# ffreyer/MonteCarlo.jl

Hardware: AMD Instinct MI355X
Metric: DQMC sweeps/sec, 16x16 Hubbard beta=8 dtau=0.1; achieved % fp64 MFMA roofline (higher is better)
Workload: dtype f64

## Files before the change

montecarlo.jl_amd/csrc/engine.cpp:

```cpp
#include <hip/hip_runtime.h>

#include <algorithm>
#include <cmath>
#include <cstdio>
#include <cstdlib>
#include <cstring>
#include <string>
#include <vector>

#include "../../include/dqmc_hip.h"
#include "kernels.h"
#include <rccl/rccl.h>

using namespace dqmc;

struct dqmc_comm {
    ncclComm_t comm = nullptr;
    int nranks = 1, rank = 0, device = 0;
};

static thread_local std::string g_create_error;

struct UTStack;

struct dqmc_handle {
    dqmc_params p{};
    int n = 0, nb = 1, N = 0, M = 0, s = 0, K = 0, W = 0, units = 0;
    long nn = 0;
    double lambda = 0, epl = 0, eml = 0;
    SweepConsts sc{};
    hipStream_t stream = nullptr;
    KernelSwitches sw;
    double *eT = nullptr, *eTinv = nullptr, *eT2 = nullptr, *eTinv2 = nullptr;
    double *eT2T = nullptr;
    bool slab = false;
    bool kron = false;
    double *kron_f = nullptr;
    int kron_fa = 0, kron_fb = 0;
    int8_t *conf = nullptr;
    double *u_stack = nullptr, *t_stack = nullptr, *d_stack = nullptr;
    std::vector<double *> su, sd, st;
    double *Ul = nullptr, *Ur = nullptr, *Tl = nullptr, *Tr = nullptr, *greens = nullptr, *greens_temp = nullptr;
    double *tmp1 = nullptr, *tmp2 = nullptr, *bufA = nullptr, *bufB = nullptr;
    struct QrSet {
        double *V = nullptr, *W = nullptr, *S = nullptr, *tau = nullptr, *winv = nullptr, *ts = nullptr;
        int *pivot = nullptr;
    } qs[1];
    double *&qrV = qs[0].V, *&qrW = qs[0].W, *&qrS = qs[0].S, *&trsm_w = qs[0].winv, *&trsm_s = qs[0].ts, *&tau = qs[0].tau;
    int *&pivot = qs[0].pivot;
    double *Dl = nullptr, *Dr = nullptr;
    hipStream_t cur = nullptr;
    double *greens_alt = nullptr, *lu_img = nullptr;
    bool sweep_fused = true;
    WalkerRng *rng = nullptr;
    DevStats *stats = nullptr;
    unsigned long long *pc_scratch = nullptr;
    std::vector<double *> uniforms;
    double *acc = nullptr;
    size_t acc_n = 0;
    int n_dirs = 0;
    int *dir_ptr = nullptr, *pair_src = nullptr, *pair_trg = nullptr;
    double *corr_per_walker = nullptr, *corr_acc = nullptr;
    int K_loc = 0;
    int *trg_of = nullptr;
    size_t pc_n = 0;
    double *pc_per_walker = nullptr, *pc_acc = nullptr;
    int K_cc = 0;
    std::vector<int> cc_trg_h;
    std::vector<double> cc_T;
    CCPlan cc;
    size_t corr_n = 0;
    int current_slice = 0, direction = 0;
    bool prepared = false;
    long long conf_version = 0;
    UTStack *ut = nullptr;
    std::string err;
    bool timing = false;
    struct Ev { hipEvent_t a, b; int fam; };
    std::vector<Ev> pending;
    std::vector<hipEvent_t> pool;
    double fam_ms[DQMC_K_COUNT] = {0};
    long long fam_n[DQMC_K_COUNT] = {0};
    std::vector<void *> allocs;
    QrCoopWorkspace qr_ws;
    int qrb_sites = 0;
    struct {
// ... 240 lines not shown
    auto exy = [&](int r, int c) {
        if (tr) std::swap(r, c);
        return fy[(r >> 3) + 8 * (c >> 3)] * fx[(r & 7) + 8 * (c & 7)];
    };
    auto ez = [&](int r, int c) { return tr ? fz[c + 8 * r] : fz[r + 8 * c]; };
    for (int mp = 0; mp < 4; ++mp)
        for (int m = 0; m < 4; ++m)
            for (int r = 0; r < 4; ++r)
                for (int lane = 0; lane < 64; ++lane)
                    img_xy[((mp * 4 + m) * 4 + r) * 64 + lane] = exy(16 * mp + (lane & 15), 16 * m + 4 * r + (lane >> 4));
    for (int q = 0; q < 4; ++q)
        for (int lane = 0; lane < 64; ++lane) {
            const int row = lane & 15, k = 4 * q + (lane >> 4);
            img_z[q * 64 + lane] = (row >> 3) == (k >> 3) ? ez(row & 7, k & 7) : 0.0;
        }
}

static void read_kernel_switches(dqmc_handle *h)
{
    KernelSwitches &k = h->sw;
    k.qr_noblocked = getenv("DQMC_QR_NOBLOCKED") != nullptr;
    if (const char *e = getenv("DQMC_QRB_SITES")) k.qrb_sites = atoi(e) & 7;
    if (const char *e = getenv("DQMC_QR_TAIL")) k.qr_tail = atoi(e) != 0;
    k.qr_sc1 = getenv("DQMC_QR_SC1") != nullptr;
    k.qr_nocoop = getenv("DQMC_QR_NOCOOP") != nullptr;
    if (const char *e = getenv("DQMC_QR_FORCE_TIMEOUT"))
        k.qr_force_timeout = strncmp(e, "step:", 5) == 0 ? 2 + atoi(e + 5) : (strncmp(e, "extra:", 6) == 0 ? 1000 + atoi(e + 6) : 1);
    k.qr_nopanel = getenv("DQMC_QR_NOPANEL") != nullptr;
    k.trsm_simple = getenv("DQMC_TRSM_SIMPLE") != nullptr;
    k.sweep_split = getenv("DQMC_SWEEP_SPLIT") != nullptr;
    k.flush_ncp2 = getenv("DQMC_FLUSH_NCP2") != nullptr;
    k.no_slab = getenv("DQMC_NO_SLAB") != nullptr;
    k.no_kron = getenv("DQMC_NO_KRON") != nullptr;
}

static int alloc_qr_workspace(dqmc_handle *h)
{
    CHK(dalloc(h, &h->qr_ws.errflag, (size_t)1));
    h->qr_ws.tail = h->sw.qr_tail;
    h->qr_ws.force_sc1 = h->sw.qr_sc1;
    h->qr_ws.no_coop = h->sw.qr_nocoop;
    h->qr_ws.no_panel = h->sw.qr_nopanel;
    h->qr_ws.force_timeout = h->sw.qr_force_timeout;
    if (h->n > 256) return 0;
    hipDeviceProp_t prop;
    HIPCHK(hipGetDeviceProperties(&prop, h->p.device_id));
    const size_t slots = (size_t)((h->units + 7) / 8) * 8 * QR_COOP_SLOTS_PER_UNIT;
    CHK(dalloc(h, &h->qr_ws.mailbox, slots * QR_COOP_SLOT));
    CHK(dalloc(h, &h->qr_ws.fb, (size_t)2));
    h->qr_ws.max_blocks = prop.multiProcessorCount * qr_coop_blocks_per_cu();
    h->qr_ws.epoch = 0;
    h->qrb_sites = 0;
    if (h->n == 256 && !h->sw.qr_noblocked) {
        const int per_cu = qrb_blocks_per_cu();
        if (per_cu >= 1 && ((h->units + 7) / 8) * 64 <= prop.multiProcessorCount * per_cu) {
            CHK(dalloc(h, (char **)&h->qr_ws.mailbox2, qrb_mailbox_bytes(h->units)));
            h->qr_ws.blk_max_blocks = prop.multiProcessorCount * per_cu;
            h->qrb_sites = h->sw.qrb_sites;
        }
    }
    return 0;
}
static int check_qr_workspace(dqmc_handle *h)
{
    if (!h->qr_ws.errflag) return 0;
    int e = 0;
// ... 144 lines not shown
static SlabArgs slab_base(dqmc_handle *h, const double *X0, long x_su, long x_sb, double *out)
{
    SlabArgs a{};
    a.n_units = h->units; a.nb = h->nb; a.nsteps = 0;
    a.X0 = X0; a.x_su = x_su; a.x_sb = x_sb;
    a.out = out; a.out_su = h->nn;
    a.conf_stride = (long)h->N * h->M;
    a.epl = h->epl; a.eml = h->eml;
    return a;
}
static void slab_step_const(dqmc_handle *h, SlabArgs &a, const double *C)
{
    SlabStep &st = a.st[a.nsteps++];
    st = SlabStep{};
    st.A = C; st.su = 0; st.sb = h->nn;
}
static void slab_step_unit(dqmc_handle *h, SlabArgs &a, const double *A)
{
    SlabStep &st = a.st[a.nsteps++];
    st = SlabStep{};
    st.A = A; st.su = h->nn; st.sb = 0;
}
static int run_slab(dqmc_handle *h, const SlabArgs &a)
{
    hipEvent_t ea, eb;
    timing_events(h, &ea, &eb);
    HIPCHK(launch_slab_chain(a, h->cur, ea, eb));
    return timing_push(h, ea, eb, DQMC_K_GEMM);
}

enum { KF_ET2 = 0, KF_ETINV2 = 1, KF_ET2T = 2, KF_ETINV2T = 3 };
static bool use_kron(const dqmc_handle *h) { return h->kron && !h->cb.on; }
static bool oop_wrap(const dqmc_handle *h) { return (h->slab || h->kron) && !h->cb.on; }
static KronArgs kron_base(dqmc_handle *h, const double *X0, double *out)
{
    KronArgs a{};
    a.n_units = h->units; a.nb = h->nb; a.nsteps = 0;
    a.X0 = X0; a.x_su = h->nn;
    a.out = out; a.out_su = h->nn;
    a.conf_stride = (long)h->N * h->M;
    a.epl = h->epl; a.eml = h->eml;
    return a;
}
static KronStep &kron_step(dqmc_handle *h, KronArgs &a, int which)
{
    KronStep &st = a.st[a.nsteps++];
    st = KronStep{};
    st.ax = h->kron_f + (size_t)which * h->nb * (h->kron_fa + h->kron_fb);
    st.ay = st.ax + (size_t)h->nb * h->kron_fa;
    return st;
}
static int run_kron(dqmc_handle *h, const KronArgs &a)
{
    hipEvent_t ea, eb;
    timing_events(h, &ea, &eb);
    if (h->n == 512) HIPCHK(launch_kron3_chain(a, h->cur, ea, eb));
    else HIPCHK(launch_kron_chain(a, h->cur, ea, eb));
    return timing_push(h, ea, eb, DQMC_K_GEMM);
}

static const int8_t *conf_slice(dqmc_handle *h, int slice) { return h->conf + (long)(slice - 1) * h->N; }
static void chain_steps(dqmc_handle *h, SlabArgs &a, int dir, int idx, int t0, int t1)
{
    for (int t = t0; t < t1; ++t) {
        SlabStep &st = a.st[a.nsteps];
        if (dir == 1) {
// ... 45 lines not shown
        const int slice = dir == 1 ? (idx - 1) * h->s + 1 + t : idx * h->s - t;
        out = (t & 1) ? h->bufB : h->bufA;
        if (h->cb.on) {
            CHK(cb_mult(h, dir == 1 ? CB_LEFT_B : CB_LEFT_BDAG, slice, X, out, t == h->s - 1 ? dslot(h, src) : nullptr));
            X = out;
            continue;
        }
        GemmArgs g = gemm_base(h, C_(h, h->eT2), dir == 1 ? 0 : 1, U_(h, X), 0, out);
        if (dir == 1) g.kscale = vs_conf(h, slice, +1);
        else { g.rowscale = vs_conf(h, slice, +1); g.row_first = 1; }
        if (t == h->s - 1) g.colscale = vs_arr(dslot(h, src), h->n);
        CHK(run_gemm(h, g));
        X = out;
    }
    const int sp = h->K + 1;
    if (udt_is_fused(h, 0)) {
        CHK(udt_fused(h, out, uslot(h, sp), dslot(h, sp), h->tmp2, 1, h->qs[0]));
    } else {
        CHK(udt_factor(h, out, dslot(h, sp), h->tmp2, 1, h->qs[0]));
        CHK(udt_formq(h, uslot(h, sp), h->qs[0], h->qs[0].winv, h->qs[0].ts));
    }
    CHK(run_gemm(h, gemm_base(h, U_(h, h->tmp2), 0, U_(h, tslot(h, src)), 0, tslot(h, sp))));
    slot_swap_spare(h, dst);
    return 0;
}
static int add_slice_sequence_left(dqmc_handle *h, int idx, bool wrap_temp = false) { return add_slice_sequence(h, +1, idx, wrap_temp); }
static int add_slice_sequence_right(dqmc_handle *h, int idx) { return add_slice_sequence(h, -1, idx, false); }

static int wrap_greens_kron(dqmc_handle *h, const double *src, double *dst, int curr_slice, int direction)
{
    const int8_t *c = conf_slice(h, direction == -1 ? curr_slice - 1 : curr_slice);
    KronArgs a = kron_base(h, src, h->bufB);
    a.transpose_out = 1;
    KronStep &s1 = kron_step(h, a, direction == -1 ? KF_ETINV2 : KF_ET2);
    if (direction == -1) { s1.post_conf = c; s1.post_sign = -1; }
    else { s1.pre_conf = c; s1.pre_sign = +1; }
    CHK(run_kron(h, a));
    KronArgs b = kron_base(h, h->bufB, dst);
    b.transpose_out = 1;
    KronStep &s2 = kron_step(h, b, direction == -1 ? KF_ET2T : KF_ETINV2T);
    if (direction == -1) { s2.post_conf = c; s2.post_sign = +1; }
    else { s2.pre_conf = c; s2.pre_sign = -1; }
    return run_kron(h, b);
}
static int wrap_greens_slab(dqmc_handle *h, const double *src, double *dst, int curr_slice, int direction)
{
    if (use_kron(h)) return wrap_greens_kron(h, src, dst, curr_slice, direction);
    if (direction == -1) {
        const int8_t *c = conf_slice(h, curr_slice - 1);
        SlabArgs a = slab_base(h, h->eT2, 0, h->nn, dst);
        slab_step_unit(h, a, src);
        slab_step_const(h, a, h->eTinv2);
        a.st[1].post_conf = c; a.st[1].post_sign = -1;
        a.col_conf = c; a.col_sign = +1;
        return run_slab(h, a);
    }
    const int8_t *c = conf_slice(h, curr_slice);
    SlabArgs a = slab_base(h, h->eTinv2, 0, h->nn, dst);
    slab_step_unit(h, a, src);
    a.st[0].pre_conf = c; a.st[0].pre_sign = -1;
    slab_step_const(h, a, h->eT2);
    a.st[1].pre_conf = c; a.st[1].pre_sign = +1;
    return run_slab(h, a);
}
static int wrap_greens_inplace(dqmc_handle *h, double *gf, int curr_slice, int direction);
static int wrap_greens(dqmc_handle *h, double **gf, int curr_slice, int direction)
// ... 46 lines not shown
{
    Timed t(h, DQMC_K_MISC);
    HIPCHK(launch_prop_check(h->n, h->nb, h->W, h->greens_temp, h->greens, h->nn, h->stats, h->pc_scratch, h->cur));
    return 0;
}

static int init_stack(dqmc_handle *h)
{
    CHK(set_identity(h, h->Ul)); CHK(set_identity(h, h->Ur));
    CHK(set_identity(h, h->Tl)); CHK(set_identity(h, h->Tr));
    CHK(set_ones(h, h->Dl)); CHK(set_ones(h, h->Dr));
    h->current_slice = 0;
    h->direction = 0;
    return 0;
}
static int build_stack(dqmc_handle *h)
{
    CHK(reset_slot(h, 0));
    for (int i = 1; i <= h->K; ++i) CHK(add_slice_sequence_left(h, i));
    h->current_slice = h->M + 1;
    h->direction = -1;
    return 0;
}

static int propagate(dqmc_handle *h)
{
    const int M = h->M, s = h->s;
    if (h->direction == 1) {
        if (h->current_slice % s == 0) {
            h->current_slice += 1;
            if (h->current_slice == 1) {
                const Udt R = slot_ref(h, 0);
                CHK(reset_slot(h, 0));
                CHK(calculate_greens_src(h, h->greens, slot_ref(h, 0), R));
            } else if (1 < h->current_slice && h->current_slice <= M) {
                const int idx = (h->current_slice - 1) / s;
                const Udt R = slot_ref(h, idx);
                const bool wt = h->p.check_propagation_error != 0, wt_slab = wt && oop_wrap(h);
                CHK(add_slice_sequence_left(h, idx, wt_slab));
                const Udt L = slot_ref(h, idx);
                if (wt && !wt_slab) {
                    CHK(copy_mat(h, h->greens_temp, h->greens));
                    CHK(wrap_greens(h, &h->greens_temp, h->current_slice - 1, 1));
                }
                if (wt_slab) {
                    std::swap(h->greens, h->greens_alt);
                    CHK(calculate_greens_src(h, h->greens, L, R));
                    CHK(prop_check(h));
                    return 0;
                }
                CHK(calculate_greens_src(h, h->greens, L, R));
                if (h->p.check_propagation_error) CHK(prop_check(h));
            } else {
                CHK(add_slice_sequence_left(h, h->K));
                h->direction = -1;
                h->current_slice = M + 1;
                CHK(propagate(h));
            }
        } else {
            CHK(wrap_greens(h, &h->greens, h->current_slice, 1));
            h->current_slice += 1;
        }
    } else {
        if ((h->current_slice - 1) % s == 0) {
            h->current_slice -= 1;
            if (h->current_slice == M) {
                const Udt L = slot_ref(h, h->K);
                CHK(reset_slot(h, h->K));
                CHK(calculate_greens_src(h, h->greens, L, slot_ref(h, h->K)));
                CHK(wrap_greens(h, &h->greens, h->current_slice + 1, -1));
            } else if (0 < h->current_slice && h->current_slice < M) {
                const int idx = h->current_slice / s + 1;
                const Udt L = slot_ref(h, idx - 1);
                CHK(add_slice_sequence_right(h, idx));
                const Udt R = slot_ref(h, idx - 1);
                if (h->p.check_propagation_error) std::swap(h->greens_temp, h->greens);
                CHK(calculate_greens_src(h, h->greens, L, R));
                if (h->p.check_propagation_error) CHK(prop_check(h));
                CHK(wrap_greens(h, &h->greens, h->current_slice + 1, -1));
            } else {
                CHK(add_slice_sequence_right(h, 1));
                h->direction = 1;
                h->current_slice = 0;
                CHK(propagate(h));
            }
        } else {
            CHK(wrap_greens(h, &h->greens, h->current_slice, -1));
            h->current_slice -= 1;
        }
    }
    return 0;
}

static int sweep_spatial_launches(dqmc_handle *h);
static int sweep_spatial(dqmc_handle *h)
{
    const int l = h->current_slice;
    if (l < 1 || l > h->M) return fail(h, DQMC_ERR_STATE, "sweep_spatial: current_slice outside 1..slices");
    CHK(sweep_spatial_launches(h));
    return 0;
}
static int sweep_spatial_launches(dqmc_handle *h)
{
    const int l = h->current_slice;
    int8_t *cslice = h->conf + (long)(l - 1) * h->N;
    h->conf_version++;
    double *cur = h->greens, *alt = h->greens_alt;
    const size_t istr = (size_t)h->units * sweep_lu_image_doubles();
    const long cstr = (long)h->N * h->M;
    hipEvent_t a, b;
    if (h->sweep_fused && h->n % 64 == 0 && h->N >= 128) {
        const int nc = h->N / 64;
        timing_events(h, &a, &b);
        HIPCHK(launch_sweep_lu(h->n, h->nb, h->W, cur, h->nn, cslice, cstr, 0, 64, h->lu_img, h->sc, h->rng, h->stats,
                               h->p.check_sign_problem, h->qr_ws.errflag, h->cur, a, b));
        CHK(timing_push(h, a, b, DQMC_K_SWEEP));
        for (int c = 1; c < nc; ++c) {
            timing_events(h, &a, &b);
            HIPCHK(launch_sweep_fused(h->n, h->nb, h->W, cur, alt, h->nn, cslice, cstr, 64 * c, 64 * (c - 1),
                                      h->lu_img + (size_t)(c & 1) * istr, h->lu_img + (size_t)((c - 1) & 1) * istr, h->sc,
                                      h->rng, h->stats, h->p.check_sign_problem, h->qr_ws.errflag, h->cur, a, b));
            CHK(timing_push(h, a, b, DQMC_K_SWEEP));
            std::swap(cur, alt);
        }
        timing_events(h, &a, &b);
        HIPCHK(launch_sweep_flush_lu(h->n, h->units, cur, alt, h->nn, 64 * (nc - 1), 64,
                                     h->lu_img + (size_t)((nc - 1) & 1) * istr, h->sw, h->cur, a, b));
        CHK(timing_push(h, a, b, DQMC_K_FLUSH));
        std::swap(cur, alt);
        if (cur != h->greens) std::swap(h->greens, h->greens_alt);
        return 0;
    }
    for (int site0 = 0; site0 < h->N; site0 += 64) {
        const int ns = std::min(64, h->N - site0);
        timing_events(h, &a, &b);
        HIPCHK(launch_sweep_lu(h->n, h->nb, h->W, cur, h->nn, cslice, cstr, site0, ns, h->lu_img, h->sc,
                               h->rng, h->stats, h->p.check_sign_problem, h->qr_ws.errflag, h->cur, a, b));
        CHK(timing_push(h, a, b, DQMC_K_SWEEP));
        timing_events(h, &a, &b);
        HIPCHK(launch_sweep_flush_lu(h->n, h->units, cur, alt, h->nn, site0, ns, h->lu_img, h->sw, h->cur, a, b));
        CHK(timing_push(h, a, b, DQMC_K_FLUSH));
        std::swap(cur, alt);
    }
    if (cur != h->greens) std::swap(h->greens, h->greens_alt);
    return 0;
}

extern "C" {

const char *dqmc_last_error(const dqmc_handle *h) { return h ? h->err.c_str() : g_create_error.c_str(); }

int dqmc_device_count(void)
{
    int c = 0;
    if (hipGetDeviceCount(&c) != hipSuccess) return 0;
    return c;
}

int dqmc_create(const dqmc_params *p, dqmc_handle **out)
{
    if (!p || !out) return fail(nullptr, DQMC_ERR_INVALID, "dqmc_create: null argument");
    *out = nullptr;
// ... 268 lines not shown
    HIPCHK(hipStreamSynchronize(h->stream));
    CHK(timing_drain(h));
    CHK(check_qr_workspace(h));
    return check_rng(h);
}
int dqmc_build_stack(dqmc_handle *h)
{
    ENTER(h);
    CHK(build_stack(h));
    h->prepared = true;
    return dqmc_synchronize(h);
}
int dqmc_prepare(dqmc_handle *h)
{
    ENTER(h);
    CHK(init_stack(h));
    CHK(build_stack(h));
    CHK(propagate(h));
    h->prepared = true;
    return dqmc_synchronize(h);
}
#define NEED_PREPARED(h) \
    if (!(h)->prepared) return fail((h), DQMC_ERR_STATE, "call dqmc_prepare or dqmc_build_stack first")
int dqmc_propagate(dqmc_handle *h)
{
    ENTER(h); NEED_PREPARED(h);
    CHK(propagate(h));
    return dqmc_synchronize(h);
}
int dqmc_sweep_spatial(dqmc_handle *h)
{
    ENTER(h); NEED_PREPARED(h);
    CHK(sweep_spatial(h));
    return dqmc_synchronize(h);
}
int dqmc_update(dqmc_handle *h)
{
    ENTER(h); NEED_PREPARED(h);
    CHK(propagate(h));
    CHK(sweep_spatial(h));
    return dqmc_synchronize(h);
}
int dqmc_sweep(dqmc_handle *h, int32_t n_sweeps)
{
    ENTER(h); NEED_PREPARED(h);
    for (int i = 0; i < n_sweeps; ++i)
        for (int u = 0; u < 2 * h->M; ++u) {
            CHK(propagate(h));
            CHK(sweep_spatial(h));
        }
    return dqmc_synchronize(h);
}
int dqmc_update_until_measure(dqmc_handle *h, int32_t *n_updates)
{
    ENTER(h); NEED_PREPARED(h);
    int cnt = 0;
    do {
        CHK(propagate(h));
        CHK(sweep_spatial(h));
        ++cnt;
    } while (!(h->current_slice == 1 && h->direction == 1));
    if (n_updates) *n_updates = cnt;
    return dqmc_synchronize(h);
}

int dqmc_get_greens_eff(dqmc_handle *h, int32_t w, double *out)
{
    ENTER(h); WALKER_OK(h, w);
    HIPCHK(hipStreamSynchronize(h->stream));
    HIPCHK(hipMemcpy(out, h->greens + (size_t)w * h->nb * h->nn, sizeof(double) * h->nb * h->nn, hipMemcpyDeviceToHost));
    return DQMC_OK;
}
int dqmc_set_greens_eff(dqmc_handle *h, int32_t w, const double *in)
{
    ENTER(h); WALKER_OK(h, w);
    HIPCHK(hipStreamSynchronize(h->stream));
    HIPCHK(hipMemcpy(h->greens + (size_t)w * h->nb * h->nn, in, sizeof(double) * h->nb * h->nn, hipMemcpyHostToDevice));
    return DQMC_OK;
}
static int true_greens(dqmc_handle *h, const double *src)
{
    if (h->cb.on) {
        CHK(cb_mult(h, CB_RIGHT_ET, 0, src, h->tmp1, nullptr));
        CHK(cb_mult(h, CB_LEFT_ETINV, 0, h->tmp1, h->tmp2, nullptr));
        return 0;
    }
    CHK(run_gemm(h, gemm_base(h, U_(h, src), 0, C_(h, h->eT), 0, h->tmp1)));
    CHK(run_gemm(h, gemm_base(h, C_(h, h->eTinv), 0, U_(h, h->tmp1), 0, h->tmp2)));
    return 0;
}
int dqmc_get_greens(dqmc_handle *h, int32_t w, double *out)
{
    ENTER(h); WALKER_OK(h, w);
    CHK(true_greens(h, h->greens));
    HIPCHK(hipStreamSynchronize(h->stream));
// ... 722 lines not shown
```

montecarlo.jl_amd/csrc/kernels.h:

```cpp
#pragma once
#include <hip/hip_runtime.h>
#include <stdint.h>

namespace dqmc {

struct VecSrc {
    int mode;
    const double *d;
    long stride;
    const int8_t *conf;
    long conf_stride;
    double cpos[2], cneg[2];
};
static inline VecSrc vs_none() { VecSrc v = {}; v.mode = 0; return v; }
static inline VecSrc vs_arr(const double *d, long stride) { VecSrc v = {}; v.mode = 1; v.d = d; v.stride = stride; return v; }
static inline VecSrc vs_inv(const double *d, long stride) { VecSrc v = {}; v.mode = 3; v.d = d; v.stride = stride; return v; }
static inline VecSrc vs_min1(const double *d, long stride) { VecSrc v = {}; v.mode = 4; v.d = d; v.stride = stride; return v; }
static inline VecSrc vs_maxinv(const double *d, long stride) { VecSrc v = {}; v.mode = 5; v.d = d; v.stride = stride; return v; }
#ifdef __HIPCC__
__device__ __forceinline__ double vs_get(const VecSrc &v, int unit, int nb, int i)
{
    if (v.mode == 1) return v.d[(long)unit * v.stride + i];
    if (v.mode == 3) return 1.0 / v.d[(long)unit * v.stride + i];
    if (v.mode == 2) {
// ... 29 lines not shown
};
hipError_t launch_gemm(const GemmArgs &g, hipStream_t s, hipEvent_t start = nullptr, hipEvent_t stop = nullptr);
constexpr int SLAB_MAX_STEPS = 10;
struct SlabStep {
    const double *A; long su, sb;
    const int8_t *pre_conf; int pre_sign;
    const int8_t *post_conf; int post_sign;
};
struct SlabArgs {
    int n_units, nb, nsteps;
    SlabStep st[SLAB_MAX_STEPS];
    const double *X0; long x_su, x_sb;
    double *out; long out_su;
    const double *col_d; long col_stride;
    const int8_t *col_conf; int col_sign;
    long conf_stride;
    double epl, eml;
};
hipError_t launch_slab_chain(const SlabArgs &a, hipStream_t s, hipEvent_t start = nullptr, hipEvent_t stop = nullptr);
struct KronStep {
    const double *ax, *ay;
    const int8_t *pre_conf; int pre_sign;
    const int8_t *post_conf; int post_sign;
};
struct KronArgs {
    int n_units, nb, nsteps;
    KronStep st[SLAB_MAX_STEPS];
    const double *X0; long x_su;
    double *out; long out_su;
    const double *col_d; long col_stride;
    int transpose_out;
    long conf_stride;
    double epl, eml;
};
hipError_t launch_kron_chain(const KronArgs &a, hipStream_t s, hipEvent_t start = nullptr, hipEvent_t stop = nullptr);
hipError_t launch_kron3_chain(const KronArgs &a, hipStream_t s, hipEvent_t start = nullptr, hipEvent_t stop = nullptr);

struct KernelSwitches {
    bool qr_noblocked = false;
    int qrb_sites = 7;
    bool qr_tail = true;
    bool qr_sc1 = false;
    bool qr_nocoop = false;
    int qr_force_timeout = 0;
    bool qr_nopanel = false;
    bool trsm_simple = false;
    bool sweep_split = false;
    bool flush_ncp2 = false;
    bool no_slab = false;
    bool no_kron = false;
};

constexpr int QR_COOP_SLOT = 528;
constexpr int QR_COOP_SLOTS_PER_UNIT = 16;
struct QrCoopWorkspace {
    double *mailbox = nullptr;
    int *errflag = nullptr;
    int *fb = nullptr;
    unsigned long long epoch = 0;
    int max_blocks = 0;
    bool tail = true;
    int force_sc1 = 0;
    int no_coop = 0;
    bool no_panel = false;
    int force_timeout = 0;
    double *mailbox2 = nullptr;
    int blk_max_blocks = 0;
};
hipError_t launch_udt_blocked(int n_units, const double *A, long strideA, double *U, long strideU, double *D, long strideD,
                              double *T, long strideT, int *pivot, QrCoopWorkspace *ws, int apply_pivot, hipStream_t s,
                              const double *B = nullptr, long strideB = 0);
size_t qrb_mailbox_bytes(int n_units);
int qrb_blocks_per_cu();
hipError_t launch_qr_pivot(int n, int n_units, double *A, long strideA, double *tau, int *pivot,
                           QrCoopWorkspace *ws, double *W, long strideW, const double **factored, hipStream_t s,
                           double *X = nullptr, long strideX = 0);
int qr_coop_blocks_per_cu();

hipError_t launch_udt_finish(int n, int n_units, double *A, long strideA, const double *F, long strideF,
                             const int *pivot, double *D, long strideD, double *V, long strideV, double *Tout,
                             long strideT, int apply_pivot, hipStream_t s);

hipError_t launch_trsm_right_upper(int n, int n_units, const double *A, long strideA, const double *T,
// ... 17 lines not shown
    DevMagStats negative_probability, propagation_error;
};
#ifdef __HIPCC__
__device__ __forceinline__ double philox_uniform(unsigned long long seed, unsigned long long index)
{
    unsigned int c0 = (unsigned int)index, c1 = (unsigned int)(index >> 32), c2 = 0u, c3 = 0u;
    unsigned int k0 = (unsigned int)seed, k1 = (unsigned int)(seed >> 32);
#pragma unroll
    for (int r = 0; r < 10; ++r) {
        const unsigned long long p0 = (unsigned long long)0xD2511F53u * c0;
        const unsigned long long p1 = (unsigned long long)0xCD9E8D57u * c2;
        const unsigned int n0 = (unsigned int)(p1 >> 32) ^ c1 ^ k0;
        const unsigned int n1 = (unsigned int)p1;
        const unsigned int n2 = (unsigned int)(p0 >> 32) ^ c3 ^ k1;
        const unsigned int n3 = (unsigned int)p0;
        c0 = n0; c1 = n1; c2 = n2; c3 = n3;
        k0 += 0x9E3779B9u;
        k1 += 0xBB67AE85u;
    }
    const unsigned long long hi = c0 >> 5, lo = c1 >> 6;
    return (double)((hi << 26) | lo) * (1.0 / 9007199254740992.0);
}

__device__ __forceinline__ void magstats_push(DevMagStats &s, double value)
{
    const double v = log10(fabs(value));
    s.max = fmax(s.max, v);
    s.min = fmin(s.min, v);
    s.sum += v;
    s.count += 1;
}
#endif
size_t sweep_lu_image_doubles();
hipError_t launch_sweep_lu(int n, int nb, int n_walkers, const double *G, long strideG, int8_t *conf_slice,
                           long conf_stride, int site0, int nsites, double *img, SweepConsts sc, WalkerRng *rng,
                           DevStats *stats, int check_sign, int *errflag, hipStream_t s,
                           hipEvent_t start = nullptr, hipEvent_t stop = nullptr);
hipError_t launch_sweep_fused(int n, int nb, int n_walkers, const double *Gin, double *Gout, long strideG,
                              int8_t *conf_slice, long conf_stride, int site0, int site0p, double *img,
                              const double *imgp, SweepConsts sc, WalkerRng *rng, DevStats *stats, int check_sign,
                              int *errflag, hipStream_t s, hipEvent_t start = nullptr, hipEvent_t stop = nullptr);

hipError_t launch_sweep_flush_lu(int n, int n_units, const double *Gin, double *Gout, long strideG, int site0,
                                 int nsites, const double *img, const KernelSwitches &sw, hipStream_t s,
                                 hipEvent_t start = nullptr, hipEvent_t stop = nullptr);

struct CbArgs {
    int n, nb, side, kmax, seq_len;
    int seq[32];
    const double *vals;
    const int *cols;
    const double *X;
    double *O;
    long strideX;
    const int8_t *conf;
    long conf_stride;
    double epl, eml;
    int pre_conf, post_conf;
    const double *pre_vec, *post_vec;
    const double *qscale;
    long qstride;
};
hipError_t launch_cb_apply(const CbArgs &a, int n_units, hipStream_t s, hipEvent_t start = nullptr,
                           hipEvent_t stop = nullptr);

hipError_t launch_set_identity(int n, int count, double *A, long stride, hipStream_t s);
// ... 47 lines not shown
```

montecarlo.jl_amd/csrc/kron.hip:

```cpp
#include "kernels.h"
#include <hip/hip_ext.h>

namespace dqmc {

typedef double d4k __attribute__((ext_vector_type(4)));
#define KR_MFMA(a, b, c) __builtin_amdgcn_mfma_f64_16x16x4f64((a), (b), (c), 0, 0, 0)

constexpr int KR_N = 256;
constexpr int KR_NC = 4;
constexpr int KR_COLS = 4 * KR_NC;
constexpr int KR_TLD = 17;
constexpr int KR_SLD = 18;
constexpr int KR_LDS_T = 4 * KR_NC * 16 * KR_TLD;
constexpr int KR_LDS_S = KR_N * KR_SLD;
constexpr int KR_LDS = KR_LDS_T > KR_LDS_S ? KR_LDS_T : KR_LDS_S;

__device__ __forceinline__ double kr_conf(int8_t c, int sign, bool bn, double epl, double eml)
{
    return (((c > 0) == (sign > 0)) != bn) ? epl : eml;
}

__global__ __launch_bounds__(256) void kron_chain_kernel(KronArgs a)
{
    __shared__ __attribute__((aligned(16))) double lds[KR_LDS];
    const int unit = blockIdx.x / (KR_N / KR_COLS), c0 = KR_COLS * (blockIdx.x % (KR_N / KR_COLS));
    if (unit >= a.n_units) return;
    const int wk = a.nb == 2 ? unit >> 1 : unit, blk = a.nb == 2 ? unit & 1 : 0;
    const bool bn = blk != 0;
    const int tid = threadIdx.x, lane = tid & 63, w = tid >> 6, g = lane >> 4, ci = lane & 15;
    const long conf_off = (long)wk * a.conf_stride;
    double *tile = lds + w * (KR_NC * 16 * KR_TLD);

    d4k v[KR_NC];
    {
        const double *x0 = a.X0 + (long)unit * a.x_su + (long)KR_N * (c0 + KR_NC * w) + ci + 16 * g;
#pragma unroll
        for (int t = 0; t < KR_NC; ++t)
#pragma unroll
            for (int r = 0; r < 4; ++r) v[t][r] = x0[KR_N * t + 64 * r];
    }
    auto idx = [&](int par, int r) { return par ? (g + 4 * r) + 16 * ci : ci + 16 * (g + 4 * r); };
    struct Ops {
        double av[4], bv[4];
        int8_t cpre[4], cpost[4];
    };
    auto request = [&](int s, Ops &o) {
        const KronStep &st = a.st[s];
        const int par = s & 1;
        const double *fx = st.ax + KR_N * blk, *fy = st.ay + KR_N * blk;
        const double *fa = par ? fx : fy, *fb = par ? fy : fx;
#pragma unroll
        for (int q = 0; q < 4; ++q) {
            o.av[q] = fa[ci + 16 * (4 * q + g)];
            o.bv[q] = fb[ci + 16 * (4 * q + g)];
        }
        const int8_t *dummy = reinterpret_cast<const int8_t *>(a.X0);
        const int8_t *pre = st.pre_conf ? st.pre_conf + conf_off : dummy, *post = st.post_conf ? st.post_conf + conf_off : dummy;
#pragma unroll
        for (int r = 0; r < 4; ++r) {
            o.cpre[r] = pre[st.pre_conf ? idx(par, r) : 0];
            o.cpost[r] = post[st.post_conf ? idx(par ^ 1, r) : 0];
        }
    };
    Ops cur, nxt;
    request(0, cur);
    double cs[KR_NC];
    {
        const double *cd = a.col_d ? a.col_d + (long)unit * a.col_stride + c0 + KR_NC * w : a.X0;
#pragma unroll
        for (int t = 0; t < KR_NC; ++t) cs[t] = cd[t];
    }

    for (int s = 0; s < a.nsteps; ++s) {
        const KronStep &st = a.st[s];
        if (st.pre_conf) {
#pragma unroll
            for (int r = 0; r < 4; ++r) {
                const double f = kr_conf(cur.cpre[r], st.pre_sign, bn, a.epl, a.eml);
#pragma unroll
                for (int t = 0; t < KR_NC; ++t) v[t][r] *= f;
            }
        }
#pragma unroll
        for (int t = 0; t < KR_NC; ++t) {
            d4k p = (d4k){0.0, 0.0, 0.0, 0.0};
#pragma unroll
            for (int q = 0; q < 4; ++q) p = KR_MFMA(cur.av[q], v[t][q], p);
#pragma unroll
            for (int r = 0; r < 4; ++r) tile[t * 16 * KR_TLD + (g + 4 * r) * KR_TLD + ci] = p[r];
        }
        request(min(s + 1, a.nsteps - 1), nxt);
        __syncthreads();
#pragma unroll
        for (int t = 0; t < KR_NC; ++t) {
            d4k q4 = (d4k){0.0, 0.0, 0.0, 0.0};
#pragma unroll
            for (int q = 0; q < 4; ++q) q4 = KR_MFMA(cur.bv[q], tile[t * 16 * KR_TLD + ci * KR_TLD + 4 * q + g], q4);
            v[t] = q4;
        }
        __syncthreads();
        if (st.post_conf) {
#pragma unroll
            for (int r = 0; r < 4; ++r) {
                const double f = kr_conf(cur.cpost[r], st.post_sign, bn, a.epl, a.eml);
#pragma unroll
                for (int t = 0; t < KR_NC; ++t) v[t][r] *= f;
            }
        }
        cur = nxt;
    }
    const int par = a.nsteps & 1;
#pragma unroll
    for (int t = 0; t < KR_NC; ++t) {
        const int cl = KR_NC * w + t;
#pragma unroll
        for (int r = 0; r < 4; ++r) {
            const int i = idx(par, r);
            lds[a.transpose_out ? i * KR_SLD + cl : cl * KR_N + i] = a.col_d ? v[t][r] * cs[t] : v[t][r];
        }
    }
    __syncthreads();
    double *o = a.out + (long)unit * a.out_su;
    if (a.transpose_out) {
#pragma unroll
        for (int k = 0; k < 8; ++k) {
            const int e = 2 * (tid + 256 * k), i = e >> 4, cl = e & 15;
            *reinterpret_cast<double2 *>(o + c0 + (long)KR_N * i + cl) = *reinterpret_cast<const double2 *>(lds + i * KR_SLD + cl);
        }
    } else {
#pragma unroll
        for (int k = 0; k < 8; ++k) {
            const int e = 2 * (tid + 256 * k);
            *reinterpret_cast<double2 *>(o + (long)KR_N * c0 + e) = *reinterpret_cast<const double2 *>(lds + e);
        }
    }
}

hipError_t launch_kron_chain(const KronArgs &a, hipStream_t s, hipEvent_t start, hipEvent_t stop)
{
    if (a.nsteps < 1 || a.nsteps > SLAB_MAX_STEPS || a.nb < 1 || a.nb > 2) return hipErrorInvalidValue;
    const dim3 grid(a.n_units * (KR_N / KR_COLS)), block(256);
    if (start) hipExtLaunchKernelGGL(kron_chain_kernel, grid, block, 0, s, start, stop, 0, a);
    else hipLaunchKernelGGL(kron_chain_kernel, grid, block, 0, s, a);
    return hipGetLastError();
}

}
```

montecarlo.jl_amd/csrc/sweep_lu.hip:

```cpp
#include "kernels.h"
#include <hip/hip_ext.h>
#include <cstdlib>

namespace dqmc {

typedef double d4 __attribute__((ext_vector_type(4)));

constexpr int LU_TILE = 256;
constexpr int LU_OFF_U = 0, LU_OFF_L = 6 * LU_TILE, LU_OFF_PT = 12 * LU_TILE, LU_OFF_Q = 16 * LU_TILE;
constexpr int LU_IMG = 20 * LU_TILE;
constexpr int LU_STRIDE = LU_IMG + 64;
__host__ __device__ constexpr int lu_pair(int K, int J)
{
    return K == 0 ? J - 1 : (K == 1 ? J + 1 : 5);
}
size_t sweep_lu_image_doubles() { return LU_STRIDE; }

__device__ __forceinline__ double readlane_d(double v, int lane)
{
    const unsigned long long u = (unsigned long long)__double_as_longlong(v);
    const unsigned lo = (unsigned)__builtin_amdgcn_readlane((int)(u & 0xffffffffull), lane);
    const unsigned hi = (unsigned)__builtin_amdgcn_readlane((int)(u >> 32), lane);
    return __longlong_as_double((long long)(((unsigned long long)hi << 32) | lo));
}
#define MFMA(a, b, c) __builtin_amdgcn_mfma_f64_16x16x4f64((a), (b), (c), 0, 0, 0)
#define DQMC_GLOBAL __attribute__((address_space(1)))
typedef const DQMC_GLOBAL double *gcdp;
typedef DQMC_GLOBAL double *gdp;
typedef double d2v __attribute__((ext_vector_type(2)));
typedef const DQMC_GLOBAL d2v *gcd2p;


constexpr int LU4_SPIN = 1 << 21;
template <int NB>
struct Lu4Smem {
    double2 aST[NB][64][64];
    double xs[NB][64];
    double strip[12][NB][2][64];
    double negv[64];
    int step[64];
    int sflag[12];
    unsigned acc16[4], neg16[4];
    int ndraw[4], exh[4];
    int abort;
};
__host__ __device__ constexpr int lu4_strip_idx(int I0, int r0, int I) { return I0 == 0 ? r0 * 2 + (I - 1) : 8 + r0; }

#define LU4_ORDER() asm volatile("" ::: "memory")
// ... 969 lines not shown
```

Before: 762.4.

## Defer final sweep flush and fold it into the following kron wrap kernel

Instead of launching a separate flush kernel for the last 64-site chunk of the spatial sweep, the pending low-rank LU update is recorded and applied inside the next kron wrap kernel, which reads the LU image and G and adds the correction before the chain steps. Anywhere else that needs the updated Green's function (measurements, propagation checks, API exits) materializes the flush explicitly, and paths that recompute greens simply discard it. This removes one kernel launch and a full read/write pass of G per slice, but it adds LDS footprint and register pressure to the wrap kernel. The PF variant of the kernel also regroups blocks across XCDs, and the bookkeeping carries state-consistency risks.

```diff
diff --git a/montecarlo.jl_amd/csrc/engine.cpp b/montecarlo.jl_amd/csrc/engine.cpp
--- a/montecarlo.jl_amd/csrc/engine.cpp
+++ b/montecarlo.jl_amd/csrc/engine.cpp
@@ -52,6 +52,11 @@
     hipStream_t cur = nullptr;
     double *greens_alt = nullptr, *lu_img = nullptr;
     bool sweep_fused = true;
+    struct PendingFlush {
+        const double *G = nullptr;
+        const double *img = nullptr;
+        int site0 = 0;
+    } pf;
     WalkerRng *rng = nullptr;
     DevStats *stats = nullptr;
     unsigned long long *pc_scratch = nullptr;
@@ -358,6 +363,7 @@
     k.flush_ncp2 = getenv("DQMC_FLUSH_NCP2") != nullptr;
     k.no_slab = getenv("DQMC_NO_SLAB") != nullptr;
     k.no_kron = getenv("DQMC_NO_KRON") != nullptr;
+    k.no_wrap_flush = getenv("DQMC_NO_WRAP_FLUSH") != nullptr;
 }
 
 static int alloc_qr_workspace(dqmc_handle *h)
@@ -568,6 +574,24 @@
 enum { KF_ET2 = 0, KF_ETINV2 = 1, KF_ET2T = 2, KF_ETINV2T = 3 };
 static bool use_kron(const dqmc_handle *h) { return h->kron && !h->cb.on; }
 static bool oop_wrap(const dqmc_handle *h) { return (h->slab || h->kron) && !h->cb.on; }
+static bool fold_wrap_flush(const dqmc_handle *h)
+{
+    return use_kron(h) && h->n == 256 && h->sweep_fused && !h->sw.no_wrap_flush;
+}
+static int materialize_pending_flush(dqmc_handle *h)
+{
+    if (!h->pf.G) return 0;
+    const dqmc_handle::PendingFlush p = h->pf;
+    h->pf = dqmc_handle::PendingFlush{};
+    if (p.G != h->greens) return fail(h, DQMC_ERR_STATE, "pending sweep update does not belong to greens");
+    hipEvent_t a, b;
+    timing_events(h, &a, &b);
+    HIPCHK(launch_sweep_flush_lu(h->n, h->units, h->greens, h->greens_alt, h->nn, p.site0, 64, p.img, h->sw, h->cur, a, b));
+    CHK(timing_push(h, a, b, DQMC_K_FLUSH));
+    std::swap(h->greens, h->greens_alt);
+    return 0;
+}
+static void discard_pending_flush(dqmc_handle *h) { h->pf = dqmc_handle::PendingFlush{}; }
 static KronArgs kron_base(dqmc_handle *h, const double *X0, double *out)
 {
     KronArgs a{};
@@ -679,6 +703,11 @@
     const int8_t *c = conf_slice(h, direction == -1 ? curr_slice - 1 : curr_slice);
     KronArgs a = kron_base(h, src, h->bufB);
     a.transpose_out = 1;
+    if (h->pf.G) {
+        if (h->pf.G != src || h->n != 256) return fail(h, DQMC_ERR_STATE, "wrap of another matrix with a sweep update pending");
+        a.pf_img = h->pf.img; a.pf_img_su = (long)sweep_lu_image_doubles(); a.pf_site0 = h->pf.site0;
+        h->pf = dqmc_handle::PendingFlush{};
+    }
     KronStep &s1 = kron_step(h, a, direction == -1 ? KF_ETINV2 : KF_ET2);
     if (direction == -1) { s1.post_conf = c; s1.post_sign = -1; }
     else { s1.pre_conf = c; s1.pre_sign = +1; }
@@ -791,6 +820,7 @@
             if (h->current_slice == 1) {
                 const Udt R = slot_ref(h, 0);
                 CHK(reset_slot(h, 0));
+                discard_pending_flush(h);
                 CHK(calculate_greens_src(h, h->greens, slot_ref(h, 0), R));
             } else if (1 < h->current_slice && h->current_slice <= M) {
                 const int idx = (h->current_slice - 1) / s;
@@ -799,6 +829,7 @@
                 CHK(add_slice_sequence_left(h, idx, wt_slab));
                 const Udt L = slot_ref(h, idx);
                 if (wt && !wt_slab) {
+                    CHK(materialize_pending_flush(h));
                     CHK(copy_mat(h, h->greens_temp, h->greens));
                     CHK(wrap_greens(h, &h->greens_temp, h->current_slice - 1, 1));
                 }
@@ -808,6 +839,7 @@
                     CHK(prop_check(h));
                     return 0;
                 }
+                discard_pending_flush(h);
                 CHK(calculate_greens_src(h, h->greens, L, R));
                 if (h->p.check_propagation_error) CHK(prop_check(h));
             } else {
@@ -826,6 +858,7 @@
             if (h->current_slice == M) {
                 const Udt L = slot_ref(h, h->K);
                 CHK(reset_slot(h, h->K));
+                discard_pending_flush(h);
                 CHK(calculate_greens_src(h, h->greens, L, slot_ref(h, h->K)));
                 CHK(wrap_greens(h, &h->greens, h->current_slice + 1, -1));
             } else if (0 < h->current_slice && h->current_slice < M) {
@@ -833,7 +866,11 @@
                 const Udt L = slot_ref(h, idx - 1);
                 CHK(add_slice_sequence_right(h, idx));
                 const Udt R = slot_ref(h, idx - 1);
-                if (h->p.check_propagation_error) std::swap(h->greens_temp, h->greens);
+                if (h->p.check_propagation_error) {
+                    CHK(materialize_pending_flush(h));
+                    std::swap(h->greens_temp, h->greens);
+                }
+                discard_pending_flush(h);
                 CHK(calculate_greens_src(h, h->greens, L, R));
                 if (h->p.check_propagation_error) CHK(prop_check(h));
                 CHK(wrap_greens(h, &h->greens, h->current_slice + 1, -1));
@@ -864,8 +901,10 @@
     const int l = h->current_slice;
     int8_t *cslice = h->conf + (long)(l - 1) * h->N;
     h->conf_version++;
+    CHK(materialize_pending_flush(h));
     double *cur = h->greens, *alt = h->greens_alt;
     const size_t istr = (size_t)h->units * sweep_lu_image_doubles();
+
     const long cstr = (long)h->N * h->M;
     hipEvent_t a, b;
     if (h->sweep_fused && h->n % 64 == 0 && h->N >= 128) {
@@ -882,11 +921,15 @@
             CHK(timing_push(h, a, b, DQMC_K_SWEEP));
             std::swap(cur, alt);
         }
-        timing_events(h, &a, &b);
-        HIPCHK(launch_sweep_flush_lu(h->n, h->units, cur, alt, h->nn, 64 * (nc - 1), 64,
-                                     h->lu_img + (size_t)((nc - 1) & 1) * istr, h->sw, h->cur, a, b));
-        CHK(timing_push(h, a, b, DQMC_K_FLUSH));
-        std::swap(cur, alt);
+        const double *img_last = h->lu_img + (size_t)((nc - 1) & 1) * istr;
+        if (fold_wrap_flush(h)) {
+            h->pf = dqmc_handle::PendingFlush{cur, img_last, 64 * (nc - 1)};
+        } else {
+            timing_events(h, &a, &b);
+            HIPCHK(launch_sweep_flush_lu(h->n, h->units, cur, alt, h->nn, 64 * (nc - 1), 64, img_last, h->sw, h->cur, a, b));
+            CHK(timing_push(h, a, b, DQMC_K_FLUSH));
+            std::swap(cur, alt);
+        }
         if (cur != h->greens) std::swap(h->greens, h->greens_alt);
         return 0;
     }
@@ -1221,6 +1264,7 @@
 {
     ENTER(h); NEED_PREPARED(h);
     CHK(sweep_spatial(h));
+    CHK(materialize_pending_flush(h));
     return dqmc_synchronize(h);
 }
 int dqmc_update(dqmc_handle *h)
@@ -1228,6 +1272,7 @@
     ENTER(h); NEED_PREPARED(h);
     CHK(propagate(h));
     CHK(sweep_spatial(h));
+    CHK(materialize_pending_flush(h));
     return dqmc_synchronize(h);
 }
 int dqmc_sweep(dqmc_handle *h, int32_t n_sweeps)
@@ -1238,6 +1283,7 @@
             CHK(propagate(h));
             CHK(sweep_spatial(h));
         }
+    CHK(materialize_pending_flush(h));
     return dqmc_synchronize(h);
 }
 int dqmc_update_until_measure(dqmc_handle *h, int32_t *n_updates)
@@ -1250,6 +1296,7 @@
         ++cnt;
     } while (!(h->current_slice == 1 && h->direction == 1));
     if (n_updates) *n_updates = cnt;
+    CHK(materialize_pending_flush(h));
     return dqmc_synchronize(h);
 }
 
diff --git a/montecarlo.jl_amd/csrc/kernels.h b/montecarlo.jl_amd/csrc/kernels.h
--- a/montecarlo.jl_amd/csrc/kernels.h
+++ b/montecarlo.jl_amd/csrc/kernels.h
@@ -85,6 +85,8 @@
     int transpose_out;
     long conf_stride;
     double epl, eml;
+    const double *pf_img; long pf_img_su;
+    int pf_site0;
 };
 hipError_t launch_kron_chain(const KronArgs &a, hipStream_t s, hipEvent_t start = nullptr, hipEvent_t stop = nullptr);
 hipError_t launch_kron3_chain(const KronArgs &a, hipStream_t s, hipEvent_t start = nullptr, hipEvent_t stop = nullptr);
@@ -102,6 +104,7 @@
     bool flush_ncp2 = false;
     bool no_slab = false;
     bool no_kron = false;
+    bool no_wrap_flush = false;
 };
 
 constexpr int QR_COOP_SLOT = 528;
@@ -185,6 +188,14 @@
 }
 #endif
 size_t sweep_lu_image_doubles();
+constexpr int LU_TILE = 256;
+constexpr int LU_OFF_U = 0, LU_OFF_L = 6 * LU_TILE, LU_OFF_PT = 12 * LU_TILE, LU_OFF_Q = 16 * LU_TILE;
+constexpr int LU_IMG = 20 * LU_TILE;
+constexpr int LU_STRIDE = LU_IMG + 64;
+__host__ __device__ constexpr int lu_pair(int K, int J)
+{
+    return K == 0 ? J - 1 : (K == 1 ? J + 1 : 5);
+}
 hipError_t launch_sweep_lu(int n, int nb, int n_walkers, const double *G, long strideG, int8_t *conf_slice,
                            long conf_stride, int site0, int nsites, double *img, SweepConsts sc, WalkerRng *rng,
                            DevStats *stats, int check_sign, int *errflag, hipStream_t s,
diff --git a/montecarlo.jl_amd/csrc/kron.hip b/montecarlo.jl_amd/csrc/kron.hip
--- a/montecarlo.jl_amd/csrc/kron.hip
+++ b/montecarlo.jl_amd/csrc/kron.hip
@@ -14,17 +14,162 @@
 constexpr int KR_LDS_T = 4 * KR_NC * 16 * KR_TLD;
 constexpr int KR_LDS_S = KR_N * KR_SLD;
 constexpr int KR_LDS = KR_LDS_T > KR_LDS_S ? KR_LDS_T : KR_LDS_S;
+constexpr int KR_PF_TS = 16 * 17;
+constexpr int KR_PF_IMG = 0, KR_PF_X = 20 * KR_PF_TS, KR_PF_R0 = KR_PF_X + 64, KR_PF_RLD = 65;
+constexpr int KR_PF_D = KR_LDS_T, KR_PF_DLD = 257;
+constexpr int KR_LDS_PF = KR_PF_D + KR_COLS * KR_PF_DLD;
+static_assert(KR_PF_R0 + KR_COLS * KR_PF_RLD <= KR_LDS_PF && KR_LDS <= KR_LDS_PF, "pending-chunk LDS layout");
+
+#define KR_GLOBAL __attribute__((address_space(1)))
+typedef const KR_GLOBAL double *kr_gcdp;
+typedef double kr_d2 __attribute__((ext_vector_type(2)));
+typedef const KR_GLOBAL kr_d2 *kr_gcd2p;
 
 __device__ __forceinline__ double kr_conf(int8_t c, int sign, bool bn, double epl, double eml)
 {
     return (((c > 0) == (sign > 0)) != bn) ? epl : eml;
 }
 
+#ifdef KR_STAMPS
+__device__ long long *kr_stamp_ptr = nullptr;
+#define KR_STAMP(k)                                                                                   \
+    do {                                                                                              \
+        if (PF && threadIdx.x == 0 && kr_stamp_ptr)                                                   \
+            kr_stamp_ptr[16 * blockIdx.x + (k)] = (long long)__builtin_amdgcn_s_memtime();            \
+    } while (0)
+#define KR_STAMP_RT(k)                                                                                \
+    do {                                                                                              \
+        if (PF && threadIdx.x == 0 && kr_stamp_ptr)                                                   \
+            kr_stamp_ptr[16 * blockIdx.x + (k)] = (long long)__builtin_amdgcn_s_memrealtime();        \
+    } while (0)
+extern "C" int dqmc_debug_kr_stamps(void *devptr)
+{
+    return (int)hipMemcpyToSymbol(HIP_SYMBOL(kr_stamp_ptr), &devptr, sizeof(void *));
+}
+#else
+#define KR_STAMP(k) do { } while (0)
+#define KR_STAMP_RT(k) do { } while (0)
+#endif
+template <bool PF>
+__device__ __forceinline__ void kr_apply_pending(const KronArgs &a, int unit, int c0, d4k (&v)[KR_NC], double *lds)
+{
+    const int tid = threadIdx.x, lane = tid & 63, w = tid >> 6, g = lane >> 4, ci = lane & 15;
+    const int site0 = a.pf_site0;
+    const kr_gcdp img = (kr_gcdp)(a.pf_img + (long)unit * a.pf_img_su);
+    const kr_gcdp G = (kr_gcdp)(a.X0 + (long)unit * a.x_su);
+    double *limg = lds + KR_PF_IMG, *lx = lds + KR_PF_X, *lr = lds + KR_PF_R0, *ld = lds + KR_PF_D;
+    constexpr int NI = LU_IMG / 2 / 256;
+    static_assert(NI * 512 == LU_IMG, "image staging");
+    kr_d2 iv[NI];
+#pragma unroll
+    for (int i = 0; i < NI; ++i) iv[i] = reinterpret_cast<kr_gcd2p>(img)[tid + 256 * i];
+    const double xin = img[LU_IMG + (tid & 63)];
+#pragma unroll
+    for (int i = 0; i < NI; ++i) {
+        const int p = 2 * (tid + 256 * i), tl = p >> 8, r = (p >> 6) & 3, ln = p & 63;
+        double *d = limg + tl * KR_PF_TS + (4 * r + (ln >> 4)) * 17 + (ln & 15);
+        d[0] = iv[i].x;
+        d[1] = iv[i].y;
+    }
+    if (tid < 64) lx[tid] = xin;
+    {
+        const int rr = site0 >> 6;
+#pragma unroll
+        for (int t = 0; t < KR_NC; ++t) {
+            const double r0 = rr == 0 ? v[t][0] : (rr == 1 ? v[t][1] : (rr == 2 ? v[t][2] : v[t][3]));
+            lr[(KR_NC * w + t) * KR_PF_RLD + ci + 16 * g] = r0;
+        }
+    }
+    __syncthreads();
+    KR_STAMP(2);
+    auto A = [&](int tl, int q) { return limg[tl * KR_PF_TS + ci * 17 + 4 * q + g]; };
+    auto xr = [&](int J, int r) { return lx[16 * J + 4 * r + g]; };
+    constexpr int TU = LU_OFF_U / LU_TILE, TL = LU_OFF_L / LU_TILE, TP = LU_OFF_PT / LU_TILE, TQ = LU_OFF_Q / LU_TILE;
+    const kr_gcdp gc = G + 64 * w + ci + (long)KR_N * (site0 + g);
+    double ca[2][4][4];
+    auto fetch = [&](int J, double (&c)[4][4]) {
+#pragma unroll
+        for (int q = 0; q < 4; ++q)
+#pragma unroll
+            for (int mm = 0; mm < 4; ++mm) c[mm][q] = gc[16 * mm + (long)KR_N * (16 * J + 4 * q)];
+    };
+    fetch(0, ca[0]);
+    d4k xv[4], rh[4];
+#pragma unroll
+    for (int J = 0; J < 4; ++J) {
+        d4k acc;
+#pragma unroll
+        for (int r = 0; r < 4; ++r) acc[r] = lr[ci * KR_PF_RLD + 16 * J + 4 * r + g];
+#pragma unroll
+        for (int K = 0; K < J; ++K)
+#pragma unroll
+            for (int q = 0; q < 4; ++q) acc = KR_MFMA(A(TL + lu_pair(K, J), q), xv[K][q], acc);
+        d4k z = (d4k){0.0, 0.0, 0.0, 0.0};
+#pragma unroll
+        for (int q = 0; q < 4; ++q) z = KR_MFMA(A(TQ + J, q), acc[q], z);
+#pragma unroll
+        for (int r = 0; r < 4; ++r) xv[J][r] = z[r] * xr(J, r);
+    }
+#pragma unroll
+    for (int J = 3; J >= 0; --J) {
+        d4k acc = (d4k){0.0, 0.0, 0.0, 0.0};
+#pragma unroll
+        for (int K = J + 1; K < 4; ++K)
+#pragma unroll
+            for (int q = 0; q < 4; ++q) acc = KR_MFMA(A(TU + lu_pair(J, K), q), rh[K][q], acc);
+#pragma unroll
+        for (int r = 0; r < 4; ++r) acc[r] = xv[J][r] + xr(J, r) * acc[r];
+        d4k o = (d4k){0.0, 0.0, 0.0, 0.0};
+#pragma unroll
+        for (int q = 0; q < 4; ++q) o = KR_MFMA(A(TP + J, q), acc[q], o);
+        rh[J] = o;
+    }
+    KR_STAMP(3);
+    d4k dm[4];
+#pragma unroll
+    for (int mm = 0; mm < 4; ++mm) dm[mm] = (d4k){0.0, 0.0, 0.0, 0.0};
+#pragma unroll
+    for (int J = 0; J < 4; ++J) {
+        if (J < 3) fetch(J + 1, ca[(J + 1) & 1]);
+        __builtin_amdgcn_sched_barrier(0);
+#pragma unroll
+        for (int q = 0; q < 4; ++q)
+#pragma unroll
+            for (int mm = 0; mm < 4; ++mm) {
+                const int i = 16 * (4 * w + mm) + ci, s = 16 * J + 4 * q + g;
+                const double c = ca[J & 1][mm][q] - (i == site0 + s ? 1.0 : 0.0);
+                dm[mm] = KR_MFMA(c, rh[J][q], dm[mm]);
+            }
+        __builtin_amdgcn_sched_barrier(0);
+    }
+    KR_STAMP(4);
+    __syncthreads();
+#pragma unroll
+    for (int mm = 0; mm < 4; ++mm)
+#pragma unroll
+        for (int r = 0; r < 4; ++r) ld[ci * KR_PF_DLD + 16 * (4 * w + mm) + 4 * r + g] = dm[mm][r];
+    __syncthreads();
+#pragma unroll
+    for (int t = 0; t < KR_NC; ++t)
+#pragma unroll
+        for (int r = 0; r < 4; ++r) v[t][r] += ld[(KR_NC * w + t) * KR_PF_DLD + ci + 16 * (g + 4 * r)];
+}
+
+template <bool PF>
 __global__ __launch_bounds__(256) void kron_chain_kernel(KronArgs a)
 {
-    __shared__ __attribute__((aligned(16))) double lds[KR_LDS];
-    const int unit = blockIdx.x / (KR_N / KR_COLS), c0 = KR_COLS * (blockIdx.x % (KR_N / KR_COLS));
+    __shared__ __attribute__((aligned(16))) double lds[PF ? KR_LDS_PF : KR_LDS];
+#ifndef KR_NO_XCD_GROUPS
+    constexpr bool XG = PF;
+#else
+    constexpr bool XG = false;
+#endif
+    const unsigned bq = XG ? blockIdx.x >> 3 : blockIdx.x;
+    const int unit = XG ? (bq / (KR_N / KR_COLS)) * 8 + (blockIdx.x & 7) : bq / (KR_N / KR_COLS);
+    const int c0 = KR_COLS * (bq % (KR_N / KR_COLS));
     if (unit >= a.n_units) return;
+    KR_STAMP(0);
+    KR_STAMP_RT(1);
     const int wk = a.nb == 2 ? unit >> 1 : unit, blk = a.nb == 2 ? unit & 1 : 0;
     const bool bn = blk != 0;
     const int tid = threadIdx.x, lane = tid & 63, w = tid >> 6, g = lane >> 4, ci = lane & 15;
@@ -70,6 +215,8 @@
 #pragma unroll
         for (int t = 0; t < KR_NC; ++t) cs[t] = cd[t];
     }
+    if constexpr (PF) kr_apply_pending<PF>(a, unit, c0, v, lds);
+    KR_STAMP(5);
 
     for (int s = 0; s < a.nsteps; ++s) {
         const KronStep &st = a.st[s];
@@ -109,6 +256,7 @@
         }
         cur = nxt;
     }
+    KR_STAMP(6);
     const int par = a.nsteps & 1;
 #pragma unroll
     for (int t = 0; t < KR_NC; ++t) {
@@ -134,14 +282,24 @@
             *reinterpret_cast<double2 *>(o + (long)KR_N * c0 + e) = *reinterpret_cast<const double2 *>(lds + e);
         }
     }
+    KR_STAMP(7);
+    KR_STAMP_RT(8);
 }
 
 hipError_t launch_kron_chain(const KronArgs &a, hipStream_t s, hipEvent_t start, hipEvent_t stop)
 {
     if (a.nsteps < 1 || a.nsteps > SLAB_MAX_STEPS || a.nb < 1 || a.nb > 2) return hipErrorInvalidValue;
+    if (a.pf_img && (a.pf_site0 < 0 || a.pf_site0 % 64 != 0 || a.pf_site0 + 64 > KR_N || a.pf_img_su < LU_STRIDE))
+        return hipErrorInvalidValue;
     const dim3 grid(a.n_units * (KR_N / KR_COLS)), block(256);
-    if (start) hipExtLaunchKernelGGL(kron_chain_kernel, grid, block, 0, s, start, stop, 0, a);
-    else hipLaunchKernelGGL(kron_chain_kernel, grid, block, 0, s, a);
+    if (a.pf_img) {
+        const dim3 gridx((a.n_units + 7) / 8 * 8 * (KR_N / KR_COLS));
+        if (start) hipExtLaunchKernelGGL(kron_chain_kernel<true>, gridx, block, 0, s, start, stop, 0, a);
+        else hipLaunchKernelGGL(kron_chain_kernel<true>, gridx, block, 0, s, a);
+    } else {
+        if (start) hipExtLaunchKernelGGL(kron_chain_kernel<false>, grid, block, 0, s, start, stop, 0, a);
+        else hipLaunchKernelGGL(kron_chain_kernel<false>, grid, block, 0, s, a);
+    }
     return hipGetLastError();
 }
 
diff --git a/montecarlo.jl_amd/csrc/sweep_lu.hip b/montecarlo.jl_amd/csrc/sweep_lu.hip
--- a/montecarlo.jl_amd/csrc/sweep_lu.hip
+++ b/montecarlo.jl_amd/csrc/sweep_lu.hip
@@ -6,14 +6,6 @@
 
 typedef double d4 __attribute__((ext_vector_type(4)));
 
-constexpr int LU_TILE = 256;
-constexpr int LU_OFF_U = 0, LU_OFF_L = 6 * LU_TILE, LU_OFF_PT = 12 * LU_TILE, LU_OFF_Q = 16 * LU_TILE;
-constexpr int LU_IMG = 20 * LU_TILE;
-constexpr int LU_STRIDE = LU_IMG + 64;
-__host__ __device__ constexpr int lu_pair(int K, int J)
-{
-    return K == 0 ? J - 1 : (K == 1 ? J + 1 : 5);
-}
 size_t sweep_lu_image_doubles() { return LU_STRIDE; }
 
 __device__ __forceinline__ double readlane_d(double v, int lane)
```

New measurement: 778.8, median of 6. 1.02x the previous value.
